# EPFL-VILAB/MultiMAE

Measured on AMD Instinct MI355X. Metric: pre-train images/sec (whole node), ViT-B RGB+D+S 224^2 98-vis-tok, higher is better.
Workload: dtype bf16 (fp32_output_adapters: fp16 storage); 1 GPU; BASELINE.json configs[2]: ViT-B, RGB+depth+semseg, 224^2, Dirichlet alpha=1.0, 98 visible tokens, 4 cross-attention decoders (dim 256, depth 2), semseg adapter (fp32_output_adapters) with fp16 STORAGE (activations / saved tensors / gradients of the adapter as IEEE half in HBM: every matmul input carries the 11-bit significand TF32 gave the reference on A100; gradients stored times a power of two f; per_gpu_batch=256, global_batch=256, parallelism=dp1

## Files before the change

### include/mmae.h

```cpp
#ifndef MMAE_H
#define MMAE_H

#include <stddef.h>
#include <stdint.h>

#ifdef __cplusplus
extern "C" {
#endif

#define MMAE_ABI_VERSION 7

#define MMAE_F32  0
#define MMAE_BF16 1
#define MMAE_F32X3 2
#define MMAE_F32F16 3
#define MMAE_MXFP8 4

#define MMAE_F16 5

#define MMAE_EINVAL   (-1)
#define MMAE_ELAUNCH  (-2)
#define MMAE_ESUPPORT (-3)

int mmae_abi_version(void);
// ... 26 lines not shown
    float alpha;
    int32_t tile;
    int32_t split_k;
    void* ws;
    int64_t ws_elems;
    float* colsum_part;
    float* a_colsum;
    int32_t a_colsum_acc;
    const void* a_scale;
    const void* b_scale;
    void* q_out; void* q_scale;
    int64_t ldq;
    const float* a_amax;
    const float* ln_gamma; const float* ln_beta; void* ln_out; float* ln_mean; float* ln_rstd; float ln_eps;
} mmae_gemm_desc;

int mmae_gemm(const mmae_gemm_desc* d, void* stream);
int mmae_gemm_plan(const mmae_gemm_desc* d, int* tile, int* split_k);
int mmae_gemm_auto_splitk(int M, int N, int K, int ab_dtype);
int mmae_gemm_cu_reserve(int k);
int mmae_gemm_cu_share(int k);
int mmae_gemm_side_cus(int k);
#ifdef MMAE_EXPERIMENTS
int mmae_gemm_duo_occupancy(int tile);
#endif

int64_t mmae_mx_scale_bytes(int rows, int cols);
int mmae_mx_quant(const void* x, int x_dtype, int64_t ldx, int rows, int cols, void* q, int64_t ldq, void* scales, void* stream);
int mmae_mx_quant_t(const void* w, int w_dtype, int64_t ldw, int n, int k, void* q, int64_t ldq, void* scales, void* stream);
int mmae_mx_quant_rows_t(const void* x, int x_dtype, int64_t ldx, int M, int C, void* q, int64_t ldq, void* scales, void* stream);
int mmae_mx_wgrad(int on);
int mmae_gelu_grad_aux(int on);
int mmae_ln_fuse(int on);
int mmae_xattn_fuse(int on);
int mmae_mx_scale_clear(void* scales, int rows, int cols, void* stream);
int mmae_layernorm_fwd_mx(const float* x, const float* gamma, const float* beta, void* y_bf16, float* mean, float* rstd, int64_t R, int D,
                          float eps, void* q, void* scales, void* stream);
int mmae_attn_fwd_mx(const void* q, const void* k, const void* v, void* o, float* lse, int B, int H, int Nq, int Nk, int hd,
                     int64_t q_sb, int64_t q_sr, int64_t k_sb, int64_t k_sr, int64_t v_sb, int64_t v_sr, int64_t o_sb, int64_t o_sr,
                     float scale, void* mx_q, void* mx_scale, void* stream);
int mmae_attn_bwd_mx(const void* q, const void* k, const void* v, const void* o, const void* d_o, const float* lse, void* dq, void* dk,
                     void* dv, int B, int H, int Nq, int Nk, int hd, int64_t q_sb, int64_t q_sr, int64_t k_sb, int64_t k_sr, int64_t v_sb,
                     int64_t v_sr, int64_t o_sb, int64_t o_sr, int64_t dq_sb, int64_t dq_sr, int64_t dk_sb, int64_t dk_sr, int64_t dv_sb,
                     int64_t dv_sr, float scale, void* mx_q, void* mx_scale, void* stream);
int64_t mmae_mx_tmp_bytes(int rows, int cols);
int mmae_mx_prepare_weights(int n, const void* const* w, int w_dtype, const int32_t* n_out, const int32_t* k_in, void* const* dst, void* stream);
int mmae_probe_mx_mfma(const int32_t* a_64x8, const int32_t* b_64x8, const int32_t* scale_a_64, const int32_t* scale_b_64, int opsel_a, int opsel_b,
                       float* out_64x16, void* stream);

int mmae_gemm_timing_enable(int on);
int mmae_gemm_timing_read(double* ms3, double* flop3, int64_t* calls3);
int mmae_gemm_timing_read_bytes(double* bytes3);

typedef struct mmae_dw_problem {
    const void* dy; int64_t ldy;
    const void* x; int64_t ldx;
    float* dw; float* db;
    int32_t n_out, k_in;
} mmae_dw_problem;

typedef struct mmae_dw_group_desc {
    int32_t n, rows, ab_dtype, accumulate, split_k;
    mmae_dw_problem p[8];
    float* ws; int64_t ws_elems;
    const float* unscale;
} mmae_dw_group_desc;
// ... 181 lines not shown
    int32_t kind, C, H, W, ph, pw, k_off;
    int32_t n_cls;
} mmae_patch_src;

int mmae_patch_rows(const mmae_patch_src* srcs_host, const int32_t* task_offsets_host, int T, const int64_t* sel,
                    void* rows, int rows_dtype, int B, int n_sel, int Ktot, void* stream);
int mmae_semseg_emb_bwd(const void* d_rows, int rows_dtype, int64_t ld, const int64_t* cls, const int64_t* sel, float* d_emb,
                        int B, int H, int W, int E, int ph, int pw, int n_sel, int k_off, int tok_off, int n_patches, int n_cls,
                        void* stream);
int64_t mmae_semseg_emb_bwd_ws_elems(int B, int n_sel, int E, int n_cls);
int mmae_semseg_emb_bwd_det(const void* d_rows, int rows_dtype, int64_t ld, const int64_t* cls, const int64_t* sel, float* d_emb,
                            int B, int H, int W, int E, int ph, int pw, int n_sel, int k_off, int tok_off, int n_patches, int n_cls,
                            float* ws, int64_t ws_elems, int accumulate, void* stream);
int mmae_tokens_assemble(float* tok, const float* proj, const float* const* bias_host, const float* const* pos_host,
                         const int32_t* task_offsets_host, int T, const int64_t* sel, const float* global_tok, int B, int n_sel,
                         int G, int D, void* stream);
int mmae_tokens_assemble_bwd_nblk(int B);
int mmae_tokens_assemble_bwd(const float* d_tok, void* d_proj, int proj_dtype, const int32_t* task_offsets_host, int T,
                             const int64_t* sel, float* part, int B, int n_sel, int G, int D, void* stream);

int mmae_patch_embed_supported(const mmae_patch_src* srcs_host, int T, int n_sel, int D);
int mmae_patch_embed_fwd(const mmae_patch_src* srcs_host, const void* const* w_bf16_host, const float* const* bias_host,
                         const float* const* pos_host, const int32_t* task_offsets_host, int T, const int64_t* sel,
                         const float* global_tok, float* tok, void* rows_bf16, int B, int n_sel, int G, int D, int Ktot, void* stream);

int mmae_decoder_build(const float* ctx, const int64_t* ids_keep, const int64_t* ids_restore,
                       const float* mask_token, const float* task_emb, const float* pos,
                       const int32_t* task_offsets_host, int T, int q_task, int B, int n_keep, int G, int D,
                       int n_q, float* queries, float* context, void* stream);
int mmae_decoder_build_bwd_nblk(int B);
int mmae_decoder_build_bwd(const float* d_queries, const float* d_context, const int64_t* ids_keep,
                           const int64_t* ids_restore, const int32_t* task_offsets_host, int T, int q_task,
                           int B, int n_keep, int G, int D, int n_q, float* d_ctx, float* part, void* stream);

int mmae_unpatchify(const float* patches, float* img, int B, int C, int nh, int nw, int ph, int pw, void* stream);
int mmae_patchify(const float* img, void* patches, int patches_dtype, int64_t ld, int B, int C, int nh, int nw, int ph,
                  int pw, void* stream);

int mmae_loss_split(void);
int mmae_masked_pixel_loss_fwd(const float* pred, const float* target, const int64_t* mask, int kind, int norm_pix,
                               int B, int C, int H, int W, int patch, float* stats, float* partial, float* per_sample,
                               float* loss, void* stream);
int mmae_masked_pixel_loss_bwd(const float* pred, const float* target, const int64_t* mask, int kind, int norm_pix,
                               int B, int C, int H, int W, int patch, const float* stats, const float* per_sample,
                               const float* loss, const float* upstream, float* d_pred, void* stream);
int mmae_masked_ce_fwd(const float* logits, const int64_t* target, const int64_t* mask, int B, int C, int H, int W,
                       int patch, float label_smoothing, float* lse, float* partial, float* per_sample, float* loss, void* stream);
int mmae_masked_ce_bwd(const float* logits, const int64_t* target, const int64_t* mask, int B, int C, int H, int W,
                       int patch, float label_smoothing, const float* lse, const float* per_sample, const float* loss,
                       const float* upstream, float* d_logits, void* stream);

int mmae_masked_pixel_loss_pat_fwd(const float* pat, const float* target, const int64_t* mask, int kind, int norm_pix, int B, int C, int H,
                                   int W, int patch, float* stats, float* partial, float* per_sample, float* loss, void* stream);
int mmae_masked_pixel_loss_pat_bwd(const float* pat, const float* target, const int64_t* mask, int kind, int norm_pix, int B, int C, int H,
                                   int W, int patch, const float* stats, const float* per_sample, const float* loss, const float* upstream,
                                   void* d_pat, int d_pat_dtype, int64_t ld_pat, float* amax, void* stream);
int mmae_masked_ce_pat_fwd(const float* pat, const int64_t* target, const int64_t* mask, int B, int C, int H, int W, int patch,
                           float label_smoothing, float* lse_pat, float* partial, float* per_sample, float* loss, void* stream);
int mmae_masked_ce_pat_bwd(const float* pat, const int64_t* target, const int64_t* mask, int B, int C, int H, int W, int patch,
                           float label_smoothing, const float* lse_pat, const float* per_sample, const float* loss, const float* upstream,
                           void* d_pat, int d_pat_dtype, int64_t ld_pat, float* amax, void* stream);

int mmae_sumsq(const float* x, int64_t n, float* out, float* ws, void* stream);
int mmae_adamw(float* p, const float* g, float* m, float* v, int64_t n, float lr, float beta1, float beta2,
               float eps, float weight_decay, int step, const float* grad_scale_dev, const int32_t* skip_flag,
               void* shadow, int shadow_dtype, void* stream);
// ... 92 lines not shown
```

### multimae_amd/csrc/composite.hip

```cpp
#include <math.h>
#include <stdlib.h>
#include <atomic>
#include <mutex>
#include "gemm_common.h"

namespace {

struct Ctx {
    int act_dtype, f32_gemm, grad_acc;
    float* ws_main; int64_t ws_main_elems;
    float* ws_side; int64_t ws_side_elems;
    void* mx_tmp = nullptr; int64_t mx_tmp_bytes = 0;
    const void* const* x3_w = nullptr; int x3_n = 0;
    void* x3_tmp = nullptr; int64_t x3_tmp_bytes = 0;
    const float* dy_amax = nullptr;
    bool b16() const { return act_dtype != MMAE_F32; }
    bool h16() const { return act_dtype == MMAE_F16; }
    int ab() const { return b16() ? act_dtype : f32_gemm; }
    int ab_grad() const { return b16() ? act_dtype : ((f32_gemm == MMAE_F32F16 && !dy_amax) ? MMAE_F32X3 : f32_gemm); }
    const float* amax_for(int ab) const { return ab == MMAE_F32F16 ? dy_amax : nullptr; }
    const float* unscale() const { return h16() ? dy_amax : nullptr; }
    size_t es() const { return b16() ? 2 : 4; }
};
inline bool is16(int act) { return act != MMAE_F32; }
// ... 35 lines not shown
int mx_in_operand(const Ctx& c, const void* x, int64_t ldx, int M, int K, int mx_in, int mx_out, const void** q, const void** s, hipStream_t st) {
    if (mx_in < 0) return mx_operand(c, x, ldx, M, K, mx_out == 0 ? 1 : 0, q, s, st);
    void *qq, *ss;
    int rc = mx_slot(c, mx_in, M, K, &qq, &ss);
    *q = qq; *s = ss;
    return rc;
}

struct EventRing {
    std::mutex mu;
    hipEvent_t ring[256];
    int made = 0, pos = 0;
    hipEvent_t next() {
        std::lock_guard<std::mutex> lk(mu);
        if (made < 256) { if (hipEventCreateWithFlags(&ring[made], hipEventDisableTiming) != hipSuccess) return nullptr; ++made; pos = made - 1; return ring[pos]; }
        pos = (pos + 1) & 255;
        return ring[pos];
    }
};
EventRing g_fork_ring, g_held_ring;

int fork_to(hipStream_t from, hipStream_t to) {
    if (from == to) return 0;
    hipEvent_t e = g_fork_ring.next();
    if (!e || hipEventRecord(e, from) != hipSuccess || hipStreamWaitEvent(to, e, 0) != hipSuccess) {
        mmae_set_error("composite: could not order one stream behind the other");
        return MMAE_ELAUNCH;
    }
    return 0;
}

struct LnSide { const float* g; const float* b; void* out; float* mean; float* rstd; float eps; };
std::atomic<int> g_ln_fuse{1};
bool ln_side_ok(const Ctx& c, int N, int K, int out_dtype) {
    return g_ln_fuse.load(std::memory_order_relaxed) != 0 && is16(c.act_dtype) && out_dtype == MMAE_F32 && N == 256 && (K % 32) == 0 && !c.x3_w;
}

int lin_fwd(const Ctx& c, const void* x, const void* w, const float* bias, void* out, int out_dtype, int M, int N, int K,
            const float* resid, void* aux, int epi, hipStream_t st, const void* const* mxw = nullptr, int mx_in = -1, int mx_out = -1,
            const LnSide* ln = nullptr) {
    mmae_gemm_desc g = {};
    if (ln) { g.ln_gamma = ln->g; g.ln_beta = ln->b; g.ln_out = ln->out; g.ln_mean = ln->mean; g.ln_rstd = ln->rstd; g.ln_eps = ln->eps; }
    g.A = x; g.B = w; g.C = out;
    g.ab_dtype = c.ab();
    g.c_dtype = out_dtype;
    g.M = M; g.N = N; g.K = K;
    g.lda = K; g.ldb = K; g.ldc = N;
    g.batch = g.batch_inner = 1;
    g.bias = bias; g.resid = resid; g.ldr = N;
    g.aux = aux; g.ldaux = N; g.aux_dtype = c.act_dtype;
    g.epi = epi; g.alpha = 1.0f;
    bool x3p = false;
    if (!mxw) {
        int rc3 = 0;
        const void* a3 = nullptr;
        const void* const* t3 = x3_operand(c, x, K, w, M, K, &a3, st, &rc3);
        if (rc3) return rc3;
        if (t3) { g.A = a3; g.B = t3[1]; g.K = 3 * K; g.lda = g.ldb = 3LL * K; g.ab_dtype = MMAE_BF16; x3p = true; }
    }
    if (mxw) {
        int rc = mx_in_operand(c, x, K, M, K, mx_in, mx_out, &g.A, &g.a_scale, st);
        if (rc) return rc;
        if (mx_out >= 0) { if ((rc = mx_slot(c, mx_out, M, N, &g.q_out, &g.q_scale))) return rc; g.ldq = N; }
        g.B = mxw[0]; g.b_scale = mxw[1]; g.ab_dtype = MMAE_MXFP8; g.split_k = 1;
        return mmae_gemm(&g, st);
    }
// ... 414 lines not shown
        void *aq, *as;
        if ((rc = mx_slot(c, 0, R, D, &aq, &as)) || (rc = attn_strides_fwd(d, st, aq, as))) return rc;
    } else if ((rc = attn_strides_fwd(d, st))) return rc;
    if (d->dp1) {
        if ((rc = lin_fwd(c, d->ao, d->proj_w, d->proj_b, d->branch, MMAE_F32, R, D, D, nullptr, nullptr, MMAE_EPI_NONE, st, mx ? mx + 4 : nullptr, pre))) return rc;
        if ((rc = mmae_rowscale_add(d->x0, d->branch, d->dp1, d->x1, R, d->N, D, st))) return rc;
    } else {
        if ((rc = lin_fwd(c, d->ao, d->proj_w, d->proj_b, d->x1, MMAE_F32, R, D, D, d->x0, nullptr, MMAE_EPI_NONE, st, mx ? mx + 4 : nullptr, pre, -1,
                          side ? &ln2s : nullptr))) return rc;
    }
    if (!side && (rc = ln(d->x1, d->n2_w, d->n2_b, d->ln2, d->mean2, d->rstd2))) return rc;
    const int hq = pre < 0 ? -1 : 1;
    if ((rc = lin_fwd(c, d->ln2, d->fc1_w, d->fc1_b, d->hact, act, R, Hd, D, nullptr, d->hpre, epi_gelu(act), st, mx ? mx + 8 : nullptr, pre, hq))) return rc;
    if (d->dp2) {
        if ((rc = lin_fwd(c, d->hact, d->fc2_w, d->fc2_b, d->branch, MMAE_F32, R, D, Hd, nullptr, nullptr, MMAE_EPI_NONE, st, mx ? mx + 12 : nullptr, hq))) return rc;
        return mmae_rowscale_add(d->x1, d->branch, d->dp2, d->x2, R, d->N, D, st);
    }
    return lin_fwd(c, d->hact, d->fc2_w, d->fc2_b, d->x2, MMAE_F32, R, D, Hd, d->x1, nullptr, MMAE_EPI_NONE, st, mx ? mx + 12 : nullptr, hq, -1,
                   (side && next) ? next : nullptr);
}

static bool block_side_ok(const mmae_block_desc& b) {
    const Ctx c = ctx_of(&b);
    return !(b.mx_w && b.act_dtype == MMAE_BF16) && !b.dp1 && !b.dp2 && ln_side_ok(c, b.D, b.D, MMAE_F32) && (b.Hd % 32) == 0;
}

std::atomic<int> g_xattn_fuse{0};
int mmae_xattn_fuse(int on) {
    const int prev = g_xattn_fuse.load(std::memory_order_relaxed);
    if (on >= 0) g_xattn_fuse.store(on ? 1 : 0, std::memory_order_relaxed);
    return prev;
}

int mmae_ln_fuse(int on) {
    const int prev = g_ln_fuse.load(std::memory_order_relaxed);
    if (on >= 0) g_ln_fuse.store(on ? 1 : 0, std::memory_order_relaxed);
    return prev;
}

int mmae_gelu_grad_aux(int on) {
    const int prev = g_gelu_grad_aux.load(std::memory_order_relaxed);
    if (on >= 0) g_gelu_grad_aux.store(on ? 1 : 0, std::memory_order_relaxed);
    return prev;
}

int mmae_mx_wgrad(int on) {
    const int prev = g_mx_wgrad.load(std::memory_order_relaxed);
    if (on >= 0) g_mx_wgrad.store(on ? 1 : 0, std::memory_order_relaxed);
    return prev;
}

int mmae_block_bwd(const mmae_block_desc* d, void* stream, void* side_stream) {
    int rc = check_desc(d);
    if (rc) return rc;
    MMAE_REQUIRE(d->dx && d->dx_act && d->dx0 && d->d_hpre && d->d_ln2 && d->d_ao && d->d_qkv && d->d_ln1 && d->dx1 && d->part1 && d->part2,
                 "block_bwd: null gradient / temporary buffer");
    const int act = d->act_dtype;
    MMAE_REQUIRE(act == MMAE_F32 || (d->dx1_act && d->dx0_act), "block_bwd: 16-bit activations need dx1_act / dx0_act");
    MMAE_REQUIRE(act != MMAE_F16 || d->dy_amax, "block_bwd: fp16 storage needs dy_amax (the scale its gradients are stored in)");
    MMAE_REQUIRE(!d->g_fc1_b || d->part_h, "block_bwd: part_h needed for the fc1 bias gradient");
    MMAE_REQUIRE(!(d->dp1 || d->dp2) || d->dxs_act, "block_bwd: stochastic depth needs the dxs_act scratch buffer");
    MMAE_REQUIRE(!(d->dp2 && d->fc2_b_done), "block_bwd: with a scaled MLP branch the fc2 bias gradient cannot come from the producer of dx");
    hipStream_t st = (hipStream_t)stream;
    hipStream_t sd = side_stream ? (hipStream_t)side_stream : st;
    const Ctx c = ctx_of(d);
    const int R = d->B * d->N, D = d->D, Hd = d->Hd, N = d->N, hd = D / d->heads;
// ... 216 lines not shown
    for (int l = 0; l < d->depth; ++l) a.blocks[l] = carve_block_act(cv, d->B, d->n_q, D, d->heads, d->Hd, es);
    a.h_act = is16(d->act_dtype) ? cv.take(Rq * D * es) : nullptr;
    a.pat = d->pat ? d->pat : cv.takeT<float>(Rq * kp_of(d));
    a.x3_tmp = adapter_x3_bytes(d) ? cv.take(adapter_x3_bytes(d)) : nullptr;
    return a;
}

struct AdapterTmp {
    void *d_pat, *dh_act, *d_hpre, *d_on, *dx_act, *d_xo, *d_q, *d_kv, *d_qn, *d_cn, *d_ctx_act;
    float *dh, *part_h, *dx, *part_o, *d_queries, *part_q, *d_context, *part_c, *d_ctx, *part_b;
    BlockTmp blocks[8];
    void* x3_tmp;
};
int64_t ldpat_of(const mmae_adapter_desc* d) { return (kp_of(d) + 7) / 8 * 8; }

AdapterTmp carve_adapter_tmp(Carver& cv, const mmae_adapter_desc* d) {
    const size_t es = es_of(d->act_dtype);
    const bool bf = is16(d->act_dtype);
    const int64_t Rq = (int64_t)d->B * d->n_q, Rc = (int64_t)d->B * d->NC;
    const int D = d->D;
    AdapterTmp t;
    t.d_pat = cv.take(Rq * ldpat_of(d) * es);
    t.dh_act = cv.take(Rq * D * es);
    t.dh = bf ? cv.takeT<float>(Rq * D) : nullptr;
    for (int l = 0; l < d->depth; ++l) t.blocks[l] = carve_block_tmp(cv, d->B, d->n_q, D, d->Hd, es, bf, false);
    t.part_h = cv.takeT<float>((Rq + 31) / 32 * d->Hd);
    t.d_hpre = cv.take(Rq * d->Hd * es); t.d_on = cv.take(Rq * D * es);
    t.dx = cv.takeT<float>(Rq * D); t.dx_act = bf ? cv.take(Rq * D * es) : nullptr;
    t.part_o = cv.takeT<float>((int64_t)mmae_layernorm_bwd_nblk(Rq) * 3 * D);
    t.d_xo = cv.take(Rq * D * es); t.d_q = cv.take(Rq * D * es); t.d_kv = cv.take(Rc * 2 * D * es);
    t.d_qn = cv.take(Rq * D * es); t.d_cn = cv.take(Rc * D * es);
    t.d_queries = cv.takeT<float>(Rq * D); t.part_q = cv.takeT<float>((int64_t)mmae_layernorm_bwd_nblk(Rq) * 3 * D);
    t.d_context = cv.takeT<float>(Rc * D); t.part_c = cv.takeT<float>((int64_t)mmae_layernorm_bwd_nblk(Rc) * 3 * D);
    t.d_ctx = cv.takeT<float>(Rc * D); t.part_b = cv.takeT<float>((int64_t)mmae_decoder_build_bwd_nblk(d->B) * (d->T + 1) * D);
    t.d_ctx_act = bf ? cv.take(Rc * D * es) : nullptr;
    t.x3_tmp = adapter_x3_bytes(d) ? cv.take(adapter_x3_bytes(d)) : nullptr;
    return t;
}

int check_adapter(const mmae_adapter_desc* d) {
    MMAE_REQUIRE(d, "adapter: null descriptor");
    MMAE_REQUIRE(d->B > 0 && d->NC > 0 && d->Denc > 0 && d->D > 0 && d->heads > 0 && d->Hd > 0 && d->D % d->heads == 0 && d->depth >= 0 &&
                 d->depth <= 8 && d->T >= 1 && d->T <= 7 && d->q_task >= -1 && d->q_task < d->T && d->G >= 0 && d->n_q > 0 && d->NC > d->G,
                 "adapter: bad geometry");
    MMAE_REQUIRE(d->C > 0 && d->nh > 0 && d->nw > 0 && d->ph > 0 && d->pw > 0 && d->nh * d->nw == d->n_q, "adapter: bad patch geometry");
    MMAE_REQUIRE(d->act_dtype == MMAE_BF16 || d->act_dtype == MMAE_F16 || (d->act_dtype == MMAE_F32 && (d->f32_gemm == MMAE_F32X3 || d->f32_gemm == MMAE_F32F16)),
                 "adapter: activations must be bf16, fp16 (MMAE_F16), or f32 with split-bf16 (MMAE_F32X3) / fp16-operand (MMAE_F32F16) products");
    if (d->act_dtype == MMAE_F16 && ((d->D % 32) || (d->Denc % 32) || (d->Hd % 32) || (kp_of(d) % 8))) {
        mmae_set_error("adapter: fp16 storage needs D, Denc, Hd multiples of 32 and C * ph * pw a multiple of 8"); return MMAE_ESUPPORT;
    }
    const int hd = d->D / d->heads;
    if ((hd != 32 && hd != 64) || d->n_q > 256 || d->NC > 256) { mmae_set_error("adapter: geometry outside the fused attention kernel"); return MMAE_ESUPPORT; }
    if (d->act_dtype == MMAE_F32) {
        const int64_t qp = (d->n_q + 31) / 32 * 32, kp = (d->NC + 31) / 32 * 32;
        if (4 * (qp + kp) * hd * 2 + 8 * qp > 160 * 1024) { mmae_set_error("adapter: f32 attention tiles exceed the LDS"); return MMAE_ESUPPORT; }
    }
    if ((d->D % 8) || (d->Denc % 8) || (d->Hd % 8) || (kp_of(d) % 4)) { mmae_set_error("adapter: widths must be multiples of 8 (patch row of 4)"); return MMAE_ESUPPORT; }
    MMAE_REQUIRE(d->task_offsets_host && d->w && d->p && d->mask_token && d->task_emb && d->pos && d->enc && d->ids_keep && d->ids_restore && d->act,
                 "adapter: null pointer");
    MMAE_REQUIRE(is16(d->act_dtype) || d->enc_act == nullptr || d->enc_act == (const void*)d->enc, "adapter: enc_act must alias enc for f32 activations");
    return 0;
}

Ctx ctx_of(const mmae_adapter_desc* d, void* x3_tmp) {
    Ctx c{d->act_dtype, d->f32_gemm, d->grad_acc, d->ws_main, d->ws_main_elems, d->ws_side, d->ws_side_elems};
    if (x3_tmp) { c.x3_w = d->x3_w; c.x3_n = d->x3_n; c.x3_tmp = x3_tmp; c.x3_tmp_bytes = adapter_x3_bytes(d); }
    c.dy_amax = d->dy_amax;
// ... 163 lines not shown
        dh = o; dh_act = oa;
        fc2_done = gb[15] != nullptr;
    }
    if ((rc = lin_dx(c, dh_act, D, f2w, t.d_hpre, act, Rq, D, Hd, a.hpre, epi_dgelu(act), gb[13] ? t.part_h : nullptr, st))) return rc;
    if ((rc = fork_to(st, sd))) return rc;
    if (!grp_q.add(dh_act, D, a.hact, Hd, gb[14], fc2_done ? nullptr : gb[15], D, Hd) &&
        (rc = lin_dw(c, dh_act, D, a.hact, gb[14], fc2_done ? nullptr : gb[15], Rq, D, Hd, sd, &cbat))) return rc;
    if ((rc = lin_dx(c, t.d_hpre, Hd, f1w, t.d_on, act, Rq, Hd, D, nullptr, MMAE_EPI_NONE, nullptr, st))) return rc;
    if (!grp_q.add(t.d_hpre, Hd, a.on, D, gb[12], nullptr, Hd, D) && (rc = lin_dw(c, t.d_hpre, Hd, a.on, gb[12], nullptr, Rq, Hd, D, sd))) return rc;
    if (gb[13] && (rc = cbat.add1(c, t.part_h, MMAE_F32, (Rq + 31) / 32, Hd, Hd, gb[13], sd))) return rc;
    if ((rc = mmae_layernorm_bwd(t.d_on, act, a.x, onw, a.omean, a.orstd, dh, t.dx, bf ? t.dx_act : nullptr, act, t.part_o, Rq, D, st))) return rc;
    const void* dx_act = bf ? (const void*)t.dx_act : (const void*)t.dx;
    if ((rc = lin_dx(c, dx_act, D, pw, t.d_xo, act, Rq, D, D, nullptr, MMAE_EPI_NONE, nullptr, st))) return rc;
    if ((rc = fork_to(st, sd))) return rc;
    if ((rc = cbat.add3(c, t.part_o, mmae_layernorm_bwd_nblk(Rq), D, gb[10], gb[11], gb[5], sd))) return rc;
    if (!grp_q.add(dx_act, D, a.xo, D, gb[4], nullptr, D, D) && (rc = lin_dw(c, dx_act, D, a.xo, gb[4], nullptr, Rq, D, D, sd))) return rc;
    {
        auto fn = act == MMAE_BF16 ? mmae_attn_bwd : (act == MMAE_F16 ? mmae_attn_bwd_f16 : mmae_attn_bwd_f32x3);
        const char* kv = (const char*)a.kv; char* dkv = (char*)t.d_kv;
        if (!bf && c.ab_grad() == MMAE_F32F16) {
            if ((rc = mmae_attn_bwd_f32f16(a.q, kv, kv + (size_t)D * es, a.xo, t.d_xo, a.lse, t.d_q, dkv, dkv + (size_t)D * es, B, d->heads, n_q, NC, hd,
                                           (int64_t)n_q * D, D, (int64_t)NC * 2 * D, 2 * D, (int64_t)NC * 2 * D, 2 * D, (int64_t)n_q * D, D, (int64_t)n_q * D, D,
                                           (int64_t)NC * 2 * D, 2 * D, (int64_t)NC * 2 * D, 2 * D, 1.0f / sqrtf((float)hd), c.dy_amax, st))) return rc;
        } else
        if ((rc = fn(a.q, kv, kv + (size_t)D * es, a.xo, t.d_xo, a.lse, t.d_q, dkv, dkv + (size_t)D * es, B, d->heads, n_q, NC, hd,
                     (int64_t)n_q * D, D, (int64_t)NC * 2 * D, 2 * D, (int64_t)NC * 2 * D, 2 * D, (int64_t)n_q * D, D, (int64_t)n_q * D, D,
                     (int64_t)NC * 2 * D, 2 * D, (int64_t)NC * 2 * D, 2 * D, 1.0f / sqrtf((float)hd), st))) return rc;
    }
    if ((rc = lin_dx(c, t.d_q, D, qw, t.d_qn, act, Rq, D, D, nullptr, MMAE_EPI_NONE, nullptr, st))) return rc;
    if ((rc = lin_dx(c, t.d_kv, 2 * D, kvw, t.d_cn, act, Rc, 2 * D, D, nullptr, MMAE_EPI_NONE, nullptr, st))) return rc;
    if ((rc = fork_to(st, sd))) return rc;
    if (!grp_q.add(t.d_q, D, a.qn, D, gb[0], gb[1], D, D) && (rc = lin_dw(c, t.d_q, D, a.qn, gb[0], gb[1], Rq, D, D, sd, &cbat))) return rc;
    if (!grp_c.add(t.d_kv, 2 * D, a.cn, D, gb[2], gb[3], 2 * D, D) && (rc = lin_dw(c, t.d_kv, 2 * D, a.cn, gb[2], gb[3], Rc, 2 * D, D, sd, &cbat))) return rc;
    if ((rc = mmae_layernorm_bwd(t.d_qn, act, a.queries, qnw, a.qmean, a.qrstd, nullptr, t.d_queries, nullptr, MMAE_F32, t.part_q, Rq, D, st))) return rc;
    if ((rc = mmae_layernorm_bwd(t.d_cn, act, a.context, cnw, a.cmean, a.crstd, nullptr, t.d_context, nullptr, MMAE_F32, t.part_c, Rc, D, st))) return rc;
    if ((rc = mmae_decoder_build_bwd(t.d_queries, t.d_context, d->ids_keep, d->ids_restore, d->task_offsets_host, T, d->q_task, B, NC - d->G, d->G, D,
                                     n_q, t.d_ctx, t.part_b, st))) return rc;
    const void* d_ctx_act = t.d_ctx;
    if (bf) { if ((rc = cast_to_act(act, t.d_ctx, t.d_ctx_act, (int64_t)Rc * D, st))) return rc; d_ctx_act = t.d_ctx_act; }
    if ((rc = fork_to(st, sd))) return rc;
    if ((rc = cbat.add3(c, t.part_q, mmae_layernorm_bwd_nblk(Rq), D, gb[8], gb[9], nullptr, sd))) return rc;
    if ((rc = cbat.add3(c, t.part_c, mmae_layernorm_bwd_nblk(Rc), D, gb[6], gb[7], nullptr, sd))) return rc;
    {
        float* dst[8];
        for (int i = 0; i < T; ++i) dst[i] = g_temb[i];
        dst[T] = g_mask;
        if ((rc = cbat.add(c, t.part_b, MMAE_F32, mmae_decoder_build_bwd_nblk(B), (T + 1) * D, (T + 1) * D, D, dst, T + 1, sd))) return rc;
    }
    if (!grp_c.add(d_ctx_act, D, enc_act, d->Denc, gtail[2], gtail[3], D, d->Denc) &&
        (rc = lin_dw(c, d_ctx_act, D, enc_act, gtail[2], gtail[3], Rc, D, d->Denc, sd, &cbat))) return rc;
    if ((rc = grp_q.flush(c, sd))) return rc;
    if ((rc = grp_c.flush(c, sd))) return rc;
    if ((rc = cbat.flush(c, sd))) return rc;
    return lin_dx(c, d_ctx_act, D, pcw, d->d_enc, MMAE_F32, Rc, D, d->Denc, nullptr, MMAE_EPI_NONE, nullptr, st);
}

}
```

### multimae_amd/csrc/tokens.hip

```cpp
#include "common.h"

namespace {

constexpr int MAX_TASKS = 8;

struct TaskTable { int off[MAX_TASKS + 1]; int T; };

__device__ __forceinline__ int task_of(const TaskTable& tt, int idx) {
    int t = 0;
#pragma unroll
    for (int i = 1; i < MAX_TASKS; ++i) if (i < tt.T && idx >= tt.off[i]) t = i;
    return t;
}

__global__ void __launch_bounds__(256) mask_sample_kernel(const long long* __restrict__ spt, const float* __restrict__ task_noise,
                                                          const float* __restrict__ all_noise, const TaskTable tt, int Ntot,
                                                          int n_keep, long long* __restrict__ mask_all,
                                                          long long* __restrict__ ids_keep, long long* __restrict__ ids_restore) {
    extern __shared__ float sm[];
    float* noise = sm;
    int* order = (int*)(sm + Ntot);
    const int b = blockIdx.x, tid = threadIdx.x;
    for (int j = tid; j < Ntot; j += 256) noise[j] = task_noise[(long long)b * Ntot + j];
    __syncthreads();
// ... 344 lines not shown
            }
        }
    }
    const int ns = tt.T + 1;
    const long long prow = (long long)blockIdx.y * gridDim.x + blockIdx.x;
    if (phases == 1) {
        if (ph == 0) {
#pragma unroll
            for (int i = 0; i < MAX_TASKS; ++i) if (i < tt.T) st4(part + (prow * ns + i) * D + c, acc[i]);
            st4(part + (prow * ns + tt.T) * D + c, acc[MAX_TASKS]);
        }
        return;
    }
    if (ph < phases) {
#pragma unroll
        for (int i = 0; i <= MAX_TASKS; ++i) red[ph][i][lane] = acc[i];
    }
    __syncthreads();
    if (ph == 0) {
#pragma unroll
        for (int i = 0; i <= MAX_TASKS; ++i) {
            if (i < tt.T || i == MAX_TASKS) {
                f32x4 t = red[0][i][lane];
                for (int p = 1; p < phases; ++p) {
#pragma unroll
                    for (int k = 0; k < 4; ++k) t[k] += red[p][i][lane][k];
                }
                st4(part + (prow * ns + (i == MAX_TASKS ? tt.T : i)) * D + c, t);
            }
        }
    }
}

__global__ void unpatchify_kernel(const float* __restrict__ pat, float* __restrict__ img, int C, int nh, int nw, int ph, int pw,
                                  long long total) {
    const long long i = (long long)blockIdx.x * blockDim.x + threadIdx.x;
    if (i >= total) return;
    const int W = nw * pw, H = nh * ph;
    const int x = (int)(i % W); long long r = i / W;
    const int y = (int)(r % H); r /= H;
    const int c = (int)(r % C); const long long b = r / C;
    const int py = y / ph, iy = y % ph, px = x / pw, ix = x % pw;
    img[i] = pat[((b * nh + py) * nw + px) * ((long long)C * ph * pw) + ((long long)c * ph + iy) * pw + ix];
}
template <typename PT>
__global__ void patchify_kernel(const float* __restrict__ img, PT* __restrict__ pat, long long ld, int C, int nh, int nw, int ph, int pw,
                                long long total) {
    const long long o = (long long)blockIdx.x * blockDim.x + threadIdx.x;
    if (o >= total) return;
    const int KP = C * ph * pw;
    const int k = (int)(o % KP); long long r = o / KP;
    const int px = (int)(r % nw); r /= nw;
    const int py = (int)(r % nh); const long long b = r / nh;
    const int c = k / (ph * pw), iy = (k / pw) % ph, ix = k % pw;
    const int W = nw * pw, H = nh * ph;
    ActT<PT>::st(pat + (o / KP) * ld + k, img[((b * C + c) * H + py * ph + iy) * W + px * pw + ix]);
}

__global__ void __launch_bounds__(256) unpatchify4_kernel(const float* __restrict__ pat, float* __restrict__ img, int C, int nh, int nw,
                                                          int ph, int pw, long long total4) {
    const long long i = (long long)blockIdx.x * 256 + threadIdx.x;
    if (i >= total4) return;
    const int qn = pw >> 2;
    const int q = (int)(i % qn); long long r = i / qn;
    const int iy = (int)(r % ph); r /= ph;
    const int c = (int)(r % C); r /= C;
// ... 313 lines not shown
        else DB_LAUNCH(float, true, *ln);
    } else DB_LAUNCH(float, false, none);
#undef DB_LAUNCH
    return mmae_check_launch("decoder_build");
}
extern "C" {

int mmae_decoder_build(const float* ctx, const int64_t* ids_keep, const int64_t* ids_restore, const float* mask_token,
                       const float* task_emb, const float* pos, const int32_t* task_offsets_host, int T, int q_task, int B,
                       int n_keep, int G, int D, int n_q, float* queries, float* context, void* stream) {
    MMAE_REQUIRE(task_emb && T >= 1 && T <= MAX_TASKS, "decoder_build: null task embedding table / bad task count");
    const float* rows[MAX_TASKS];
    for (int t = 0; t < T; ++t) rows[t] = task_emb + (long long)t * D;
    return mmae_decoder_build_rows(ctx, ids_keep, ids_restore, mask_token, rows, pos, task_offsets_host, T, q_task, B, n_keep, G, D, n_q,
                                   queries, context, stream);
}

static int dbb_split(int B) { return B <= 512 ? 4 : 1; }
int mmae_decoder_build_bwd_nblk(int B) { return (B < 1024 ? B : 1024) * dbb_split(B); }

int mmae_decoder_build_bwd(const float* d_queries, const float* d_context, const int64_t* ids_keep, const int64_t* ids_restore,
                           const int32_t* task_offsets_host, int T, int q_task, int B, int n_keep, int G, int D, int n_q,
                           float* d_ctx, float* part, void* stream) {
    MMAE_REQUIRE(d_queries && d_context && ids_keep && ids_restore && d_ctx && part, "decoder_build_bwd: null pointer");
    MMAE_REQUIRE(D % 4 == 0 && D <= 1024 && B > 0, "decoder_build_bwd: bad sizes");
    TaskTable tt;
    MMAE_REQUIRE(fill_tt(tt, task_offsets_host, T) == 0 && q_task >= -1 && q_task < T, "decoder_build_bwd: bad task table");
    hipLaunchKernelGGL(decoder_build_bwd_kernel, dim3(B < 1024 ? B : 1024, dbb_split(B)), dim3(256), 0, (hipStream_t)stream, d_queries,
                       d_context, (const long long*)ids_keep, (const long long*)ids_restore, tt, q_task, B, n_keep, G, D, n_q,
                       tt.off[T], d_ctx, part);
    return mmae_check_launch("decoder_build_bwd");
}

int mmae_unpatchify(const float* patches, float* img, int B, int C, int nh, int nw, int ph, int pw, void* stream) {
    MMAE_REQUIRE(patches && img && B > 0 && C > 0, "unpatchify: bad argument");
    const long long total = (long long)B * C * nh * ph * nw * pw;
    const int cbu = (pw % 4 == 0 && pw < 16) ? patch_tile_cb(ph, nw * pw) : 0;
    if (cbu > 0 && ((uintptr_t)patches % 16 == 0) && ((uintptr_t)img % 16 == 0)) {
        const long long nblk = (long long)B * nh * ((C + cbu - 1) / cbu);
        hipLaunchKernelGGL((patch_tile_kernel<float, false>), dim3((unsigned)nblk), dim3(256), (size_t)cbu * ph * nw * pw * 4, (hipStream_t)stream,
                           patches, img, (long long)C * ph * pw, C, nh, nw, ph, pw, cbu);
        return mmae_check_launch("unpatchify");
    }
    if (pw % 4 == 0 && ((uintptr_t)patches % 16 == 0) && ((uintptr_t)img % 16 == 0))
        hipLaunchKernelGGL(unpatchify4_kernel, dim3((unsigned)cdiv64(total / 4, 256)), dim3(256), 0, (hipStream_t)stream, patches, img, C,
                           nh, nw, ph, pw, total / 4);
    else
        hipLaunchKernelGGL(unpatchify_kernel, dim3((unsigned)cdiv64(total, 256)), dim3(256), 0, (hipStream_t)stream, patches, img, C, nh, nw,
                           ph, pw, total);
    return mmae_check_launch("unpatchify");
}

int mmae_patchify(const float* img, void* patches, int patches_dtype, int64_t ld, int B, int C, int nh, int nw, int ph, int pw, void* stream) {
    MMAE_REQUIRE(patches && img && B > 0 && C > 0 && ld >= (int64_t)C * ph * pw, "patchify: bad argument");
    const long long total = (long long)B * C * nh * ph * nw * pw;
    hipStream_t st = (hipStream_t)stream;
    const int cbp = (pw % 4 == 0 && pw < 16 && ld % 4 == 0) ? patch_tile_cb(ph, nw * pw) : 0;
    if (cbp > 0 && ((uintptr_t)patches % 16 == 0) && ((uintptr_t)img % 16 == 0)) {
        const dim3 grid((unsigned)((long long)B * nh * ((C + cbp - 1) / cbp)));
        const size_t lds = (size_t)cbp * ph * nw * pw * 4;
        if (patches_dtype == MMAE_BF16) hipLaunchKernelGGL((patch_tile_kernel<uint16_t, true>), grid, dim3(256), lds, st, img, (uint16_t*)patches, (long long)ld, C, nh, nw, ph, pw, cbp);
        else hipLaunchKernelGGL((patch_tile_kernel<float, true>), grid, dim3(256), lds, st, img, (float*)patches, (long long)ld, C, nh, nw, ph, pw, cbp);
        return mmae_check_launch("patchify");
    }
    if (pw % 4 == 0 && ld % 4 == 0 && ((uintptr_t)patches % 16 == 0) && ((uintptr_t)img % 16 == 0)) {
        const dim3 grid((unsigned)cdiv64(total / 4, 256));
// ... 47 lines not shown
```

### multimae_amd/ops.py

```python
from __future__ import annotations

import ctypes
import math
from typing import Optional, Sequence

import torch

from . import _lib
import contextlib

from ._lib import BF16, F16, F32, F32X3, F32F16, MXFP8, EPI_NONE, EPI_GELU, EPI_DGELU, EPI_GELU_G, EPI_MUL, AdapterDesc, BlockDesc, DwGroupDesc, GemmDesc, OptDesc, OptGroupsDesc, PatchSrc, StackDesc, check

Tensor = torch.Tensor


def _require_gpu(t: Tensor, name: str = 'tensor') -> None:
    if not t.is_cuda:
        raise RuntimeError(f'multimae_amd: {name} is on {t.device}; the engine runs on MI355X HIP kernels only '
                           '(no CPU / PyTorch fallback). Move the model and inputs to a GPU.')


def dcode(dtype: torch.dtype) -> int:
    if dtype == torch.float32:
        return F32
# ... 177 lines not shown
            q_out: Optional[MxTensor] = None, split_k: int = 1, accumulate: bool = False) -> Tensor:
    assert a.cols == b.cols, (a.cols, b.cols)
    M, N, K = a.rows, b.rows, a.cols
    d = GemmDesc()
    d.A, d.B, d.C = a.q.data_ptr(), b.q.data_ptr(), C.data_ptr()
    d.a_scale, d.b_scale = a.scales.data_ptr(), b.scales.data_ptr()
    d.ab_dtype, d.c_dtype = MXFP8, dcode(C.dtype)
    d.M, d.N, d.K = M, N, K
    d.lda, d.ldb, d.ldc = K, K, N
    d.batch = d.batch_inner = 1
    d.bias = _p(bias)
    d.resid, d.ldr = _p(resid), N
    d.aux, d.ldaux = _p(aux), N
    d.aux_dtype = dcode(aux.dtype) if aux is not None else F32
    d.epi, d.alpha, d.split_k = epi, 1.0, split_k
    d.accumulate = int(accumulate)
    if split_k > 1:
        ws = stream_workspace(_stream(), C.device, max(_WS_ELEMS[0], split_k * M * N))
        d.ws, d.ws_elems = ws.data_ptr(), ws.numel()
    d.colsum_part = _p(colsum_part)
    if q_out is not None:
        assert q_out.rows == M and q_out.cols == N
        d.q_out, d.q_scale, d.ldq = q_out.q.data_ptr(), q_out.scales.data_ptr(), N
    check(_lib.load().mmae_gemm(ctypes.byref(d), _stream()), 'mmae_gemm(mxfp8)')
    return C


def gemm_cu_reserve(k: Optional[int] = None) -> int:
    return int(_lib.load().mmae_gemm_cu_reserve(-1 if k is None else int(k)))


def ln_fuse(on: Optional[bool] = None) -> bool:
    return bool(_lib.load().mmae_ln_fuse(-1 if on is None else int(bool(on))))


def xattn_fuse(on: Optional[bool] = None) -> bool:
    return bool(_lib.load().mmae_xattn_fuse(-1 if on is None else int(bool(on))))


def gemm_cu_share(k: Optional[int] = None) -> int:
    return int(_lib.load().mmae_gemm_cu_share(-1 if k is None else int(k)))


def gemm_side_cus(k: Optional[int] = None) -> int:
    return int(_lib.load().mmae_gemm_side_cus(-1 if k is None else int(k)))


def linear_fwd(x: Tensor, w: Tensor, bias: Optional[Tensor], out: Tensor, *, resid: Optional[Tensor] = None,
               aux: Optional[Tensor] = None, epi: int = EPI_NONE, tile: int = 0, ln: Optional[tuple] = None) -> Tensor:
    M, K = x.shape
    N = w.shape[0]
    gemm(x, w, out, M, N, K, lda=K, ldb=K, ldc=N, bias=bias, resid=resid, ldr=N, aux=aux, ldaux=N, epi=epi, tile=tile, ln=ln)
    return out


def linear_dx(dy: Tensor, w: Tensor, out: Tensor, *, aux: Optional[Tensor] = None, epi: int = EPI_NONE,
              colsum_out: Optional[Tensor] = None, colsum_part: Optional[Tensor] = None, tile: int = 0) -> Tensor:
    M, N = dy.shape
    K = w.shape[1]
    part = colsum_part
    if colsum_out is not None and part is None:
        part = torch.empty(dx_colsum_part_shape(M, K), device=dy.device, dtype=torch.float32)
    gemm(dy, w, out, M, K, N, lda=dy.stride(0), ldb=K, ldc=K, b_trans=True, aux=aux, ldaux=K, epi=epi, colsum_part=part, tile=tile)
    if colsum_out is not None:
        colsum(part, colsum_out, False)
    return out
# ... 1197 lines not shown
```

Measured before the change: 8959 images/s.

## Fuse decoder query/context LayerNorm backward into decoder-build backward kernel

```diff
diff --git a/include/mmae.h b/include/mmae.h
--- a/include/mmae.h
+++ b/include/mmae.h
@@ -82,6 +82,7 @@
 int mmae_mx_wgrad(int on);
 int mmae_gelu_grad_aux(int on);
 int mmae_ln_fuse(int on);
+int mmae_ln_bwd_fuse(int on);
 int mmae_xattn_fuse(int on);
 int mmae_mx_scale_clear(void* scales, int rows, int cols, void* stream);
 int mmae_layernorm_fwd_mx(const float* x, const float* gamma, const float* beta, void* y_bf16, float* mean, float* rstd, int64_t R, int D,
@@ -329,6 +330,11 @@
 int mmae_decoder_build_bwd(const float* d_queries, const float* d_context, const int64_t* ids_keep,
                            const int64_t* ids_restore, const int32_t* task_offsets_host, int T, int q_task,
                            int B, int n_keep, int G, int D, int n_q, float* d_ctx, float* part, void* stream);
+int mmae_decoder_build_ln_bwd(const void* d_qn, const void* d_cn, int dtype, const float* queries, const float* context,
+                              const float* qmean, const float* qrstd, const float* cmean, const float* crstd,
+                              const float* q_gamma, const float* c_gamma, const int64_t* ids_keep, const int64_t* ids_restore,
+                              const int32_t* task_offsets_host, int T, int q_task, int B, int n_keep, int G, int D, int n_q,
+                              float* d_ctx, void* d_ctx_act, float* part, void* stream);
 
 int mmae_unpatchify(const float* patches, float* img, int B, int C, int nh, int nw, int ph, int pw, void* stream);
 int mmae_patchify(const float* img, void* patches, int patches_dtype, int64_t ld, int B, int C, int nh, int nw, int ph,
diff --git a/multimae_amd/csrc/composite.hip b/multimae_amd/csrc/composite.hip
--- a/multimae_amd/csrc/composite.hip
+++ b/multimae_amd/csrc/composite.hip
@@ -91,6 +91,7 @@
 
 struct LnSide { const float* g; const float* b; void* out; float* mean; float* rstd; float eps; };
 std::atomic<int> g_ln_fuse{1};
+std::atomic<int> g_ln_bwd_fuse{1};
 bool ln_side_ok(const Ctx& c, int N, int K, int out_dtype) {
     return g_ln_fuse.load(std::memory_order_relaxed) != 0 && is16(c.act_dtype) && out_dtype == MMAE_F32 && N == 256 && (K % 32) == 0 && !c.x3_w;
 }
@@ -571,6 +572,12 @@
     return prev;
 }
 
+int mmae_ln_bwd_fuse(int on) {
+    const int prev = g_ln_bwd_fuse.load(std::memory_order_relaxed);
+    if (on >= 0) g_ln_bwd_fuse.store(on ? 1 : 0, std::memory_order_relaxed);
+    return prev;
+}
+
 int mmae_ln_fuse(int on) {
     const int prev = g_ln_fuse.load(std::memory_order_relaxed);
     if (on >= 0) g_ln_fuse.store(on ? 1 : 0, std::memory_order_relaxed);
@@ -853,7 +860,7 @@
     t.d_qn = cv.take(Rq * D * es); t.d_cn = cv.take(Rc * D * es);
     t.d_queries = cv.takeT<float>(Rq * D); t.part_q = cv.takeT<float>((int64_t)mmae_layernorm_bwd_nblk(Rq) * 3 * D);
     t.d_context = cv.takeT<float>(Rc * D); t.part_c = cv.takeT<float>((int64_t)mmae_layernorm_bwd_nblk(Rc) * 3 * D);
-    t.d_ctx = cv.takeT<float>(Rc * D); t.part_b = cv.takeT<float>((int64_t)mmae_decoder_build_bwd_nblk(d->B) * (d->T + 1) * D);
+    t.d_ctx = cv.takeT<float>(Rc * D); t.part_b = cv.takeT<float>((int64_t)mmae_decoder_build_bwd_nblk(d->B) * (d->T + 5) * D);
     t.d_ctx_act = bf ? cv.take(Rc * D * es) : nullptr;
     t.x3_tmp = adapter_x3_bytes(d) ? cv.take(adapter_x3_bytes(d)) : nullptr;
     return t;
@@ -1083,20 +1090,35 @@
     if ((rc = fork_to(st, sd))) return rc;
     if (!grp_q.add(t.d_q, D, a.qn, D, gb[0], gb[1], D, D) && (rc = lin_dw(c, t.d_q, D, a.qn, gb[0], gb[1], Rq, D, D, sd, &cbat))) return rc;
     if (!grp_c.add(t.d_kv, 2 * D, a.cn, D, gb[2], gb[3], 2 * D, D) && (rc = lin_dw(c, t.d_kv, 2 * D, a.cn, gb[2], gb[3], Rc, 2 * D, D, sd, &cbat))) return rc;
+    const bool bfuse = g_ln_bwd_fuse.load(std::memory_order_relaxed) != 0 && bf && D == 256;
+    const void* d_ctx_act = t.d_ctx;
+    if (bfuse) {
+        if ((rc = mmae_decoder_build_ln_bwd(t.d_qn, t.d_cn, act, a.queries, a.context, a.qmean, a.qrstd, a.cmean, a.crstd, qnw, cnw, d->ids_keep,
+                                            d->ids_restore, d->task_offsets_host, T, d->q_task, B, NC - d->G, d->G, D, n_q, nullptr, t.d_ctx_act,
+                                            t.part_b, st))) return rc;
+        d_ctx_act = t.d_ctx_act;
+    } else {
     if ((rc = mmae_layernorm_bwd(t.d_qn, act, a.queries, qnw, a.qmean, a.qrstd, nullptr, t.d_queries, nullptr, MMAE_F32, t.part_q, Rq, D, st))) return rc;
     if ((rc = mmae_layernorm_bwd(t.d_cn, act, a.context, cnw, a.cmean, a.crstd, nullptr, t.d_context, nullptr, MMAE_F32, t.part_c, Rc, D, st))) return rc;
     if ((rc = mmae_decoder_build_bwd(t.d_queries, t.d_context, d->ids_keep, d->ids_restore, d->task_offsets_host, T, d->q_task, B, NC - d->G, d->G, D,
                                      n_q, t.d_ctx, t.part_b, st))) return rc;
-    const void* d_ctx_act = t.d_ctx;
     if (bf) { if ((rc = cast_to_act(act, t.d_ctx, t.d_ctx_act, (int64_t)Rc * D, st))) return rc; d_ctx_act = t.d_ctx_act; }
+    }
     if ((rc = fork_to(st, sd))) return rc;
-    if ((rc = cbat.add3(c, t.part_q, mmae_layernorm_bwd_nblk(Rq), D, gb[8], gb[9], nullptr, sd))) return rc;
-    if ((rc = cbat.add3(c, t.part_c, mmae_layernorm_bwd_nblk(Rc), D, gb[6], gb[7], nullptr, sd))) return rc;
     {
         float* dst[8];
         for (int i = 0; i < T; ++i) dst[i] = g_temb[i];
         dst[T] = g_mask;
-        if ((rc = cbat.add(c, t.part_b, MMAE_F32, mmae_decoder_build_bwd_nblk(B), (T + 1) * D, (T + 1) * D, D, dst, T + 1, sd))) return rc;
+        const int nb = mmae_decoder_build_bwd_nblk(B);
+        if (bfuse) {
+            float* lnd[4] = {gb[8], gb[9], gb[6], gb[7]};
+            if ((rc = cbat.add(c, t.part_b, MMAE_F32, nb, (T + 1) * D, (T + 5) * D, D, dst, T + 1, sd))) return rc;
+            if ((rc = cbat.add(c, t.part_b + (T + 1) * D, MMAE_F32, nb, 4 * D, (T + 5) * D, D, lnd, 4, sd))) return rc;
+        } else {
+            if ((rc = cbat.add3(c, t.part_q, mmae_layernorm_bwd_nblk(Rq), D, gb[8], gb[9], nullptr, sd))) return rc;
+            if ((rc = cbat.add3(c, t.part_c, mmae_layernorm_bwd_nblk(Rc), D, gb[6], gb[7], nullptr, sd))) return rc;
+            if ((rc = cbat.add(c, t.part_b, MMAE_F32, nb, (T + 1) * D, (T + 1) * D, D, dst, T + 1, sd))) return rc;
+        }
     }
     if (!grp_c.add(d_ctx_act, D, enc_act, d->Denc, gtail[2], gtail[3], D, d->Denc) &&
         (rc = lin_dw(c, d_ctx_act, D, enc_act, gtail[2], gtail[3], Rc, D, d->Denc, sd, &cbat))) return rc;
diff --git a/multimae_amd/csrc/tokens.hip b/multimae_amd/csrc/tokens.hip
--- a/multimae_amd/csrc/tokens.hip
+++ b/multimae_amd/csrc/tokens.hip
@@ -400,6 +400,115 @@
     }
 }
 
+template <bool ACC>
+__device__ __forceinline__ f32x4 build_ln_bwd_row(const f32x4 d, const f32x4 xv, float mu, float rs, const f32x4 g, f32x4& dg, f32x4& db) {
+    f32x4 xh, dh;
+    float s1 = 0.f, s2 = 0.f;
+#pragma unroll
+    for (int j = 0; j < 4; ++j) {
+        xh[j] = (xv[j] - mu) * rs;
+        dh[j] = d[j] * g[j];
+        s1 += dh[j];
+        s2 += dh[j] * xh[j];
+        if (ACC) { dg[j] += d[j] * xh[j]; db[j] += d[j]; }
+    }
+    const float c1 = wave_sum(s1) / 256.f, c2 = wave_sum(s2) / 256.f;
+    f32x4 o;
+#pragma unroll
+    for (int j = 0; j < 4; ++j) o[j] = rs * (dh[j] - c1 - xh[j] * c2);
+    return o;
+}
+
+template <typename DT>
+__global__ void __launch_bounds__(256) decoder_build_ln_bwd_kernel(const DT* __restrict__ d_qn, const DT* __restrict__ d_cn,
+                                                                   const float* __restrict__ queries, const float* __restrict__ context,
+                                                                   const float* __restrict__ qmean, const float* __restrict__ qrstd,
+                                                                   const float* __restrict__ cmean, const float* __restrict__ crstd,
+                                                                   const float* __restrict__ qgamma, const float* __restrict__ cgamma,
+                                                                   const long long* __restrict__ ids_keep, const long long* __restrict__ ids_restore,
+                                                                   const TaskTable tt, int q_task, int B, int n_keep, int G, int n_q, int Ntot,
+                                                                   float* __restrict__ d_ctx, DT* __restrict__ d_ctx_act, float* __restrict__ part) {
+    constexpr int D = 256;
+    __shared__ f32x4 tsum[4][MAX_TASKS + 1][64];
+    const int ph = __builtin_amdgcn_readfirstlane(threadIdx.x >> 6), lane = threadIdx.x & 63;
+    const int c = lane * 4;
+    const int NC = n_keep + G, NR = NC + n_q;
+    const int split = gridDim.y;
+#pragma unroll
+    for (int i = 0; i <= MAX_TASKS; ++i) tsum[ph][i][lane] = f32x4{0.f, 0.f, 0.f, 0.f};
+    f32x4 dgq = {0.f, 0.f, 0.f, 0.f}, dbq = dgq, dgc = dgq, dbc = dgq;
+    const f32x4 gq = ld4(qgamma + c), gc = ld4(cgamma + c);
+    const int stride = 4 * split, first = blockIdx.y * 4 + ph;
+    auto tadd = [&](int slot, const f32x4& v) {
+        f32x4 t = tsum[ph][slot][lane];
+#pragma unroll
+        for (int k = 0; k < 4; ++k) t[k] += v[k];
+        tsum[ph][slot][lane] = t;
+    };
+    for (int b = blockIdx.x; b < B; b += gridDim.x) {
+        f32x4 nd = {0.f, 0.f, 0.f, 0.f}, nx = nd;
+        float nmu = 0.f, nrs = 0.f;
+        int nid = 0;
+#pragma unroll 1
+        for (int rr = first - stride; rr < NR; rr += stride) {
+            const f32x4 d = nd, xv = nx;
+            const float mu = nmu, rs = nrs;
+            const int id = __builtin_amdgcn_readfirstlane(nid);
+            const int rn = rr + stride;
+            if (rn < NC) {
+                const long long row = (long long)b * NC + rn;
+                nd = ld4(d_cn + row * D + c); nx = ld4(context + row * D + c);
+                nmu = cmean[row]; nrs = crstd[row];
+                nid = rn < n_keep ? (int)ids_keep[(long long)b * n_keep + rn] : -1;
+            } else if (rn < NR) {
+                const int j = rn - NC;
+                const long long row = (long long)b * n_q + j;
+                nd = ld4(d_qn + row * D + c); nx = ld4(queries + row * D + c);
+                nmu = qmean[row]; nrs = qrstd[row];
+                nid = q_task >= 0 ? (int)ids_restore[(long long)b * Ntot + tt.off[q_task] + j] : n_keep;
+            }
+            if (rr < first) continue;
+            if (rr < NC) {
+                f32x4 v = build_ln_bwd_row<true>(d, xv, mu, rs, gc, dgc, dbc);
+                if (rr < n_keep) {
+                    const int t = task_of(tt, id);
+                    tadd(t, v);
+                    if (t == q_task) {
+                        const long long qrow = (long long)b * n_q + (id - tt.off[t]);
+                        f32x4 none = {0.f, 0.f, 0.f, 0.f};
+                        const f32x4 q = build_ln_bwd_row<false>(ld4(d_qn + qrow * D + c), ld4(queries + qrow * D + c), qmean[qrow], qrstd[qrow], gq, none, none);
+#pragma unroll
+                        for (int k = 0; k < 4; ++k) v[k] += q[k];
+                    }
+                }
+                const long long row = (long long)b * NC + rr;
+                if (d_ctx) st4(d_ctx + row * D + c, v);
+                if (d_ctx_act) st4(d_ctx_act + row * D + c, v);
+            } else {
+                const f32x4 q = build_ln_bwd_row<true>(d, xv, mu, rs, gq, dgq, dbq);
+                if (q_task >= 0) tadd(q_task, q);
+                if (!(q_task >= 0 && id < n_keep)) tadd(MAX_TASKS, q);
+            }
+        }
+    }
+    const int ns = tt.T + 5;
+    float* prow = part + ((long long)blockIdx.y * gridDim.x + blockIdx.x) * ns * D + c;
+    auto sum4 = [&](int i) {
+        const f32x4 t0 = tsum[0][i][lane], t1 = tsum[1][i][lane], t2 = tsum[2][i][lane], t3 = tsum[3][i][lane];
+        f32x4 t;
+#pragma unroll
+        for (int k = 0; k < 4; ++k) t[k] = (t0[k] + t1[k]) + (t2[k] + t3[k]);
+        return t;
+    };
+    __syncthreads();
+    for (int i = ph; i <= MAX_TASKS; i += 4)
+        if (i < tt.T || i == MAX_TASKS) st4(prow + (i == MAX_TASKS ? tt.T : i) * D, sum4(i));
+    __syncthreads();
+    tsum[ph][0][lane] = dgq; tsum[ph][1][lane] = dbq; tsum[ph][2][lane] = dgc; tsum[ph][3][lane] = dbc;
+    __syncthreads();
+    st4(prow + (tt.T + 1 + ph) * D, sum4(ph));
+}
+
 __global__ void unpatchify_kernel(const float* __restrict__ pat, float* __restrict__ img, int C, int nh, int nw, int ph, int pw,
                                   long long total) {
     const long long i = (long long)blockIdx.x * blockDim.x + threadIdx.x;
@@ -779,6 +888,28 @@
     return mmae_check_launch("decoder_build_bwd");
 }
 
+int mmae_decoder_build_ln_bwd(const void* d_qn, const void* d_cn, int dtype, const float* queries, const float* context, const float* qmean,
+                              const float* qrstd, const float* cmean, const float* crstd, const float* q_gamma, const float* c_gamma,
+                              const int64_t* ids_keep, const int64_t* ids_restore, const int32_t* task_offsets_host, int T, int q_task, int B,
+                              int n_keep, int G, int D, int n_q, float* d_ctx, void* d_ctx_act, float* part, void* stream) {
+    MMAE_REQUIRE(d_qn && d_cn && queries && context && qmean && qrstd && cmean && crstd && q_gamma && c_gamma && ids_keep && ids_restore && part,
+                 "decoder_build_ln_bwd: null pointer");
+    MMAE_REQUIRE(d_ctx || d_ctx_act, "decoder_build_ln_bwd: no destination");
+    MMAE_REQUIRE(dtype == MMAE_BF16 || dtype == MMAE_F16, "decoder_build_ln_bwd: gradients must be bf16 or fp16");
+    if (D != 256) { mmae_set_error("decoder_build_ln_bwd: a wave holds a row only at D = 256"); return MMAE_ESUPPORT; }
+    MMAE_REQUIRE(B > 0 && n_keep > 0 && G >= 0 && n_q > 0, "decoder_build_ln_bwd: bad sizes");
+    TaskTable tt;
+    MMAE_REQUIRE(fill_tt(tt, task_offsets_host, T) == 0 && q_task >= -1 && q_task < T, "decoder_build_ln_bwd: bad task table");
+    const dim3 grid(B < 1024 ? B : 1024, dbb_split(B)), block(256);
+#define DBLB(DT)                                                                                                                          \
+    hipLaunchKernelGGL((decoder_build_ln_bwd_kernel<DT>), grid, block, 0, (hipStream_t)stream, (const DT*)d_qn, (const DT*)d_cn, queries, \
+                       context, qmean, qrstd, cmean, crstd, q_gamma, c_gamma, (const long long*)ids_keep, (const long long*)ids_restore,  \
+                       tt, q_task, B, n_keep, G, n_q, tt.off[T], d_ctx, (DT*)d_ctx_act, part)
+    if (dtype == MMAE_BF16) DBLB(uint16_t); else DBLB(h16_t);
+#undef DBLB
+    return mmae_check_launch("decoder_build_ln_bwd");
+}
+
 int mmae_unpatchify(const float* patches, float* img, int B, int C, int nh, int nw, int ph, int pw, void* stream) {
     MMAE_REQUIRE(patches && img && B > 0 && C > 0, "unpatchify: bad argument");
     const long long total = (long long)B * C * nh * ph * nw * pw;
diff --git a/multimae_amd/ops.py b/multimae_amd/ops.py
--- a/multimae_amd/ops.py
+++ b/multimae_amd/ops.py
@@ -233,6 +233,10 @@
 
 def ln_fuse(on: Optional[bool] = None) -> bool:
     return bool(_lib.load().mmae_ln_fuse(-1 if on is None else int(bool(on))))
+
+
+def ln_bwd_fuse(on: Optional[bool] = None) -> bool:
+    return bool(_lib.load().mmae_ln_bwd_fuse(-1 if on is None else int(bool(on))))
 
 
 def xattn_fuse(on: Optional[bool] = None) -> bool:
```

New measurement: 9023 images/s (median of 6 runs). No clear change (+0.7%).
